# lis-epfl/apg_trajectory_tracking

Hardware: AMD Instinct MI355X
Metric: env-steps/sec (fwd+bwd through dynamics), quad horizon=10 batch=65536 (higher is better)
Workload: dtype f32; 1 GPU; quadrotor concurrent rollout fwd+bwd (dynamics + quad_mpc_loss + adjoint), BASELINE configs[1]; batch_per_gpu=65536, global_batch=65536, horizon=10, layout=packed, buffer_sets=20, input_bytes_all_sets=587202560, grad_state0=False, loss_mode=deferred, launch=hip-graph replays of the K steps, <= 1000 steps per graph, replays=3, parallelism=batch-sharded x1, no data-path collective

## Files before the change

apg_trajectory_tracking_amd/csrc/mlp_concurrent.hip:

```cpp
#include "mlp_concurrent_fwd.h"

namespace apg {
namespace {
template <bool ROWS>
__global__ __launch_bounds__(kThreads) void mlp_concurrent_bwd_tm_kernel(WgArgs A) {
  extern __shared__ __attribute__((aligned(16))) float lds_f[];
  char *lds = reinterpret_cast<char *>(lds_f);
  const int lane = threadIdx.x & 63, hi = lane >> 5, row = lane & 31;
  const int wave = __builtin_amdgcn_readfirstlane(threadIdx.x >> 6);
  const int b0 = blockIdx.x * kTrajPerBlock;
  const int b = b0 + wave * 32 + row;
  const int B = A.B;
  const bool live = b < B;
  const unsigned pN = (unsigned)B * 4u;
  const Planes Pact(A.acts, kActPlanes, pN), Pdz(A.d_zout, kNA, pN);
  const unsigned vb = live ? (unsigned)b * 4u : kDead;
  const unsigned vr = live ? vb + (hi ? 4u * pN : 0u) : kDead;
  const unsigned wcol = (unsigned)(b0 + wave * 32) * 4u;
  const unsigned vt = (unsigned)row * pN + (unsigned)hi * 16u;
  const int nw = B - (b0 + wave * 32);
  float *part = A.part + (size_t)blockIdx.x * kSlotsTm * 1024;
  char *lane_blk = lds + lane * 4;
  TmMeta &meta = *reinterpret_cast<TmMeta *>(lds + tMeta);
  bool bad = false;
// ... 210 lines not shown
      if (hi == 0)
        __builtin_nontemporal_store(
            bad ? __builtin_nanf("") : __builtin_amdgcn_ldexpf(sb, e_ - kPreD),
            bias_part + bias_id * 64 + 32 * mb + row);
      split16(v, 0, ad[mb]);
    }
  };
  auto layer64 = [&](f32x16 (&dl)[2], f32x16 (&nx)[2], int e_, int tab, int x_plane,
                     int region, int bias_id, int next_plane, int phase) {
    Op16 x[4];
    const int ex = scaled_split64(dl, x);
    Op16 ad[2][2];
    transposed_operands(x, ex, e_, bias_id, ad);
#pragma unroll
    for (int nb = 0; nb < 2; ++nb) {
      float xv[16];
      tx.get(xv);
      tx.load(Pact, vt, (unsigned)(nb == 0 ? x_plane + 32 : next_plane) * pN + wcol);
      Op16 bx[2];
      split16(xv, -kPreX, bx);
#pragma unroll
      for (int mb = 0; mb < 2; ++mb) {
        f32x16 acc;
#pragma unroll
        for (int i = 0; i < 16; ++i) acc[i] = 0.f;
#pragma unroll
        for (int kk = 0; kk < 2; ++kk) acc = mma3(ad[mb][kk], bx[kk], acc);
        add_block(lane_blk + region + (2 * nb + mb) * 4096, acc);
      }
      if (nb == 0) load_hv(x_plane);
    }
    zero(nx);
    dense64T_16(nx, x, L16, 0, tab);
#pragma unroll
    for (int rb = 0; rb < 2; ++rb)
#pragma unroll
      for (int i = 0; i < 16; ++i)
        nx[rb][i] = __builtin_amdgcn_ldexpf(nx[rb][i], ex) * (1.f - hv[rb][i] * hv[rb][i]);
    post(nx, phase + 1);
  };
  const int e3 = wg_exp(meta.dmax[1], bad);
  layer64(d, e, e3, w3, pH2, tRB, 1, pH1, 1);
  __syncthreads();
  flush_region(lds, tRB, 4 * 1024, part + sFc3 * 1024, e3, true, bad);
  zero_region(lds, tF1a, tRA - tF1a);
  const int e2 = wg_exp(meta.dmax[2], bad);
  layer64(e, d, e2, w2, pH1, tRA, 2, pX1, 2);
  __syncthreads();
  flush_region(lds, tRA, 4 * 1024, part + sFc2 * 1024, e2, false, bad);

  const int e1 = wg_exp(meta.dmax[3], bad);
  const int es = e1 + ns, ec = e1 + nc;
  {
    Op16 x1s[4];
    const int ex1 = scaled_split64(d, x1s);
    Op16 ad[2][2];
    transposed_operands(x1s, ex1, e1, 3, ad);
    Op16 bfeat[2], binr[3][2];
    if (ROWS) {
      const int bw = b0 + wave * 32 + row;
      const long long r_ = A.index[bw < B ? bw : B - 1];
      const unsigned rf = row_offset(r_, A.n_rows, A.ld_feat);
      const unsigned ri = row_offset(r_, A.n_rows, A.ld_in_ref);
      const auto sf = __builtin_amdgcn_make_buffer_rsrc(const_cast<float *>(A.r_feat), 0,
                                                        (int)A.bytes_feat, 0x00020000);
      const auto si = __builtin_amdgcn_make_buffer_rsrc(const_cast<float *>(A.r_in_ref), 0,
                                                        (int)A.bytes_in_ref, 0x00020000);
      float v[16];
      const auto rows_block = [&](__amdgpu_buffer_rsrc_t rs, unsigned rbase, int col, bool on) {
#pragma unroll
        for (int g = 0; g < 4; ++g)
#pragma unroll
          for (int c = 0; c < 4; ++c) {
            const unsigned a0 = (unsigned)__builtin_amdgcn_readlane((int)rbase, c + 8 * g),
                           a1 = (unsigned)__builtin_amdgcn_readlane((int)rbase, c + 8 * g + 4);
            const unsigned a = hi ? a1 : a0;
            const unsigned off = on && a != kDead ? a + 4u * (unsigned)col : kDead;
            v[4 * g + c] = __builtin_bit_cast(
                float, __builtin_amdgcn_raw_buffer_load_b32(rs, (int)off, 0, APG_PLANES_LD_AUX));
          }
      };
      rows_block(sf, rf, row, row < kNF);
#pragma unroll
      for (int i = 0; i < 16; ++i) v[i] = row == kNF ? 1.f : v[i];
      split16(v, ff - kPreX, bfeat);
#pragma unroll
      for (int jb = 0; jb < 3; ++jb) {
        rows_block(si, ri, 32 * jb + row, 32 * jb + row < kH * kRD);
        split16(v, fi - kPreXc, binr[jb]);
      }
    } else {
      TBlock tf;
      tf.load(Pact, row < kNF ? vt : kDead, (unsigned)pFeat * pN + wcol);
      float v[16];
      tf.get(v);
#pragma unroll
      for (int i = 0; i < 16; ++i) v[i] = row == kNF ? 1.f : v[i];
      split16(v, ff - kPreX, bfeat);
#pragma unroll
      for (int jb = 0; jb < 3; ++jb) {
        tf.load(Pact, 32 * jb + row < kH * kRD ? vt : kDead,
                (unsigned)(pInr + 32 * jb) * pN + wcol);
        tf.get(v);
        split16(v, fi - kPreXc, binr[jb]);
      }
    }
// ... 382 lines not shown
```

apg_trajectory_tracking_amd/csrc/mlp_rollout.hip:

```cpp
#include "mlp_common.h"
#include "quad_flight.h"

namespace apg {
namespace {
template <bool XMAX, bool LEGACY = false>
__global__ __launch_bounds__(kThreads) void mlp_rollout_fwd_kernel(FwdArgs A) {
  extern __shared__ __attribute__((aligned(16))) float lds[];
  fill_lds(lds, A.tables, kCfLds);
  const LdsView16 L16(lds, threadIdx.x & 63);
  const int lane = threadIdx.x & 63, hi = lane >> 5;
  const LdsView L(lds, lane);
  const int wave = __builtin_amdgcn_readfirstlane(threadIdx.x >> 6);
  const int b = (blockIdx.x * (kThreads / 64) + wave) * 32 + (lane & 31);
  const int B = A.B;
  const bool live = b < B;
  const bool st_lo = live && hi == 0;
  const unsigned pitchB = (unsigned)B * 4u, pitchN = pitchB * kH;
  const QuadConst c = A.c;
  const Planes Ps0(A.state0, 12, pitchB), Pin(A.in_ref, 2 * kH * kRD, pitchB);
  const Planes Pst(A.states, kH * 12, pitchB), Pac(A.actions, kH * 4, pitchB);
  const Planes Pfe(A.feat, kNF, pitchN), Px1(A.x1, kN1, pitchN);
  const Planes Ph(A.h, 3 * kW, pitchN), Pmk(A.mask, 5, pitchN);
  const unsigned vb = live ? (unsigned)b * 4u : kDead;
  const unsigned vb_lo = st_lo ? vb : kDead;

  float s[12];
#pragma unroll
  for (int i = 0; i < 12; ++i) s[i] = Ps0.ld(vb, i * pitchB);
  const unsigned vwin = live ? vb + (hi ? 4u * pitchB : 0u) : kDead;
  float w[kH][5];
#pragma unroll
  for (int r = 0; r < kH; ++r)
#pragma unroll
    for (int j = 0; j < 5; ++j) w[r][j] = Pin.ld(vwin, (r * kRD + j) * pitchB);
  float wmax_raw = 0.f;
  if (XMAX) {
#pragma unroll
    for (int r = 0; r < kH; ++r)
#pragma unroll
      for (int j = 0; j < 5; ++j) wmax_raw = fmaxf(wmax_raw, fabsf(w[r][j]));
  }

#pragma unroll 1
  for (int k = 0; k < kH; ++k) {
    const unsigned pB = opaque(pitchB), pN = opaque(pitchN);
    const unsigned col = (unsigned)b * 4u + (unsigned)k * pitchB;
    const unsigned vn = live ? col : kDead;
    const unsigned vn_lo = st_lo ? col : kDead;
    const unsigned vr = live ? col + (hi ? 4u * pitchN : 0u) : kDead;
    const unsigned vc = live ? col + (hi ? 32u * pitchN : 0u) : kDead;
    const unsigned vm = live ? col + (hi ? pitchN : 0u) : kDead;
    const Trig t = make_trig(&s[3]);
    float feat[kNF];
    quad_features(s, t, feat);
#pragma unroll
    for (int j = 0; j < kNF; ++j) Pfe.st(vn_lo, j * pN, feat[j]);
    float xm_c = 0.f;
    if (XMAX) {
      float xm_f = 0.f;
#pragma unroll
      for (int j = 0; j < kNF; ++j) xm_f = fmaxf(xm_f, fabsf(feat[j]));
      const float xm_i = wmax_raw + (hi ? 0.f : fmaxf(fmaxf(fabsf(s[0]), fabsf(s[1])), fabsf(s[2])));
      const float rf = wave_fmax(xm_f), ri = wave_fmax(xm_i);
      if (lane == 0) {
        float *q = A.xmax + ((size_t)(blockIdx.x * (kThreads / 64) + wave) * kH + k) * 4;
        q[1] = rf, q[2] = ri;
      }
    }

    f32x16 u[2], a[2];
    init_bias(u, L, hTbs);
    {
      float v[8];
#pragma unroll
      for (int j = 0; j < 8; ++j)
        v[j] = hi ? (8 + j < kNF ? feat[8 + j < kNF ? 8 + j : 0] : 0.f) : feat[j];
      const Op16 x = split8(v);
      u[0] = mma3(L16.A(hA, nS + 0), x, u[0]);
      u[1] = mma3(L16.A(hA, nS + 1), x, u[1]);
    }
    float sub[3] = {hi ? 0.f : s[0], hi ? 0.f : s[1], hi ? 0.f : s[2]};
    if (LEGACY) {
#pragma unroll
      for (int r = 0; r < kH; ++r)
#pragma unroll
        for (int j = 0; j < 3; ++j) w[r][j] -= sub[j];
      sub[0] = sub[1] = sub[2] = 0.f;
    }
    init_bias(a, L, hTb1);
    unsigned mbits[3] = {0u, 0u, 0u};
#pragma unroll
    for (int pp = 0; pp < kNP / 2; ++pp) {
      float rv[24];
      unsigned ws[4][5];
#pragma unroll
      for (int r = 0; r < 4; ++r)
#pragma unroll
        for (int j = 0; j < 5; ++j) {
          const float xv = j < 3 ? w[2 * pp + r][j] - sub[j] : w[2 * pp + r][j];
          const _Float16 vh = (_Float16)xv, vl = (_Float16)(xv - (float)vh);
          const h16x2 pr = {vh, vl};
          ws[r][j] = __builtin_bit_cast(unsigned, pr);
        }
#pragma unroll
// ... 224 lines not shown
    for (int sft = 32; sft >= 1; sft >>= 1) sum = fmaxf(sum, __shfl_xor(sum, sft, 64));
    if ((t & 63) == 0) wmax[t >> 6] = sum;
    __syncthreads();
    if (t < 2) {
      const float m = t ? fmaxf(fmaxf(wmax[1], wmax[2]), wmax[3]) : wmax[0];
      A.dst[kCfLds + kArTabFloats + t] =
          m > 0.f && m < 3.0e38f ? (float)__builtin_amdgcn_frexp_expf(m) : 0.f;
    }
    return;
  }
  if ((int)blockIdx.x < fwd_blocks) {
    pack_cfwd(A, blockIdx.x * blockDim.x + threadIdx.x, fwd_blocks * blockDim.x);
    return;
  }
  const int tid = (blockIdx.x - fwd_blocks) * blockDim.x + threadIdx.x;
  const int T = (gridDim.x - 1 - fwd_blocks) * blockDim.x;
  float *dstf = A.dst + kCfLds;
  unsigned *dst = reinterpret_cast<unsigned *>(dstf);
  for (int idx = tid; idx < aBlocks * 64 * 4; idx += T) {
    const int q = idx & 3, l = (idx >> 2) & 63, n = idx >> 8;
    const float w0 = car_weight(A.pol, n, l & 31, 2 * q, l >> 5);
    const float w1 = car_weight(A.pol, n, l & 31, 2 * q + 1, l >> 5);
    unsigned h, lo;
    split_pair(w0, w1, h, lo);
    dst[(gA + n * kBlock16) / 4 + l * 4 + q] = h;
    dst[(gA + n * kBlock16 + 1024) / 4 + l * 4 + q] = lo;
  }
  const ApgMlpPolicy &p = A.pol;
  for (int idx = tid; idx < 256; idx += T) {
    const int hi = idx & 1, i = (idx >> 1) & 15, rb = (idx >> 5) & 1, j = idx >> 6;
    dstf[gTo + idx] = p.w_out[j * kW + rb * 32 + rrow(i) + 4 * hi];
  }
  for (int idx = tid; idx < kNC * 3; idx += T) {
    const int ch = idx / 3, q = idx % 3;
    dstf[gAq + idx] = p.conv_w[ch * 27 + q * 3] + p.conv_w[ch * 27 + q * 3 + 1] +
                      p.conv_w[ch * 27 + q * 3 + 2];
  }
}

struct ArTmArgs {
  const float *state0, *states, *actions, *ref, *in_ref;
  const float *feat, *x1, *h;
  const unsigned *mask;
  float *loss_partials;
  float *part;
  float *grad_state0;
  const float *tables;
  const float *xmax;
  QuadConst c;
  ApgQuadLossWeights w;
  int B, ref_cols, vel_col;
};

__device__ __forceinline__ void ar_sink(const f32x16 &acc) {
  float s_ = 0.f;
#pragma unroll
  for (int i = 0; i < 16; ++i) s_ += acc[i];
  asm volatile("" ::"v"(s_));
}
__device__ __forceinline__ void ar_barrier() {
  if (APG_AR_KNOCKOUT & 16) return;
  __syncthreads();
}

struct ArMeta {
  unsigned dmax[5][8];
};
static_assert(rMeta + (int)sizeof(ArMeta) <= kLdsAll, "LDS map");

__global__ __launch_bounds__(kThreads) void mlp_rollout_bwd_tm_kernel(ArTmArgs A) {
  extern __shared__ __attribute__((aligned(16))) float lds_f[];
  char *lds = reinterpret_cast<char *>(lds_f);
  const int lane = threadIdx.x & 63, hi = lane >> 5, row = lane & 31;
  const int wave = __builtin_amdgcn_readfirstlane(threadIdx.x >> 6);
  const int b0 = blockIdx.x * kTrajPerBlock;
  const int b = b0 + wave * 32 + row;
  const int B = A.B;
  const bool live = b < B, st_lo = live && hi == 0;
  const unsigned pitchB = (unsigned)B * 4u, pitchN = pitchB * kH;
  const QuadConst c = A.c;
  const Planes Ps0(A.state0, 12, pitchB), Pst(A.states, kH * 12, pitchB);
  const Planes Pac(A.actions, kH * 4, pitchB), Prf(A.ref, kH * A.ref_cols, pitchB);
  const Planes Pin(A.in_ref, 2 * kH * kRD, pitchB);
  const Planes Pfe(A.feat, kNF, pitchN), Px1(A.x1, kN1, pitchN), Ph(A.h, 3 * kW, pitchN);
  const Planes Pmk(A.mask, 5, pitchN);
  const unsigned vb = live ? (unsigned)b * 4u : kDead;
  const unsigned wcolB = (unsigned)(b0 + wave * 32) * 4u;
  const unsigned vtN = (unsigned)row * pitchN + (unsigned)hi * 16u;
  const unsigned vtB = (unsigned)row * pitchB + (unsigned)hi * 16u;
  const __amdgpu_buffer_rsrc_t part = __builtin_amdgcn_make_buffer_rsrc(
      A.part + (size_t)blockIdx.x * kSlotsTm * 1024, 0, kSlotsTm * 4096, 0x00020000);
  char *lane_blk = lds + lane * 4;
  ArMeta &meta = *reinterpret_cast<ArMeta *>(lds + rMeta);
  const int ns = (int)A.tables[kArTabFloats];
  bool bad = false;

  zero_region(lds, rX, rMeta - rX);
  {
    const u32x4 z = {0u, 0u, 0u, 0u};
#pragma unroll
    for (int m = 0; m < kSlotsTm * 256; m += kThreads)
      __builtin_amdgcn_raw_buffer_store_b128(z, part, (int)(threadIdx.x * 16u), m * 16, 0);
  }
  fill_lds_issue(lds_f, A.tables, kArTabFloats);
  asm volatile("s_waitcnt vmcnt(0)" ::: "memory");
  __syncthreads();
  const LdsView16 L16(lds, lane);
  const LdsView L(lds_f, lane);
  float lam[12];
#pragma unroll
  for (int i = 0; i < 12; ++i) lam[i] = 0.f;
  float loss = 0.f;
  int rg = rX, ro = rY;
  int e5 = 0, ecv = 0;
  TBlock tx, tx2;
  const auto post = [&](const f32x16 (&v)[2], int phase) {
    unsigned am = 0u;
#pragma unroll
    for (int rb = 0; rb < 2; ++rb)
#pragma unroll
      for (int i = 0; i < 16; ++i) am = umax_abs(am, v[rb][i]);
    am = wave_umax(am);
    if (lane == 0) meta.dmax[phase][wave] = am;
  };
  const unsigned bias_soff = (unsigned)(uBias + (wave >> 2)) * 4096u + (unsigned)(wave & 3) * 1024u;
  const auto flush_tail = [&]() {
    flush_add<4 * 1024>(lds, rg, part, (sFc1 + 10) * 4096, e5, bad);
    flush_add<1024>(lds, rConv, part, uConv * 4096, ecv, bad, kFixConv);
  };

#pragma unroll 1
  for (int k = kH - 1; k >= 0; --k) {
    const unsigned pB = (APG_AR_KNOCKOUT & 64) ? 256u : opaque(pitchB), pN = opaque(pitchN);
    const unsigned col = (unsigned)b * 4u + (unsigned)k * pitchB;
    const unsigned vn = live ? ((APG_AR_KNOCKOUT & 64) ? (unsigned)lane * 4u : col) : kDead;
    const unsigned wcolN = wcolB + (unsigned)k * pB;
    u32x4 ident[2];
    {
      int lane_o = lane;
      asm volatile("" : "+v"(lane_o));
      ident_operands(lane_o, ident);
    }
    float dz[4];
    unsigned m0 = 0u;
    f32x16 d[2], e[2];
    float x3[2][16];
    {
      float sn[12], sc[12], a[4], rp[3], rv[3];
#pragma unroll
      for (int i = 0; i < 12; ++i) {
        sn[i] = Pst.ld(vb, (k * 12 + i) * pB);
        sc[i] = k > 0 ? Pst.ld(vb, ((k - 1) * 12 + i) * pB) : Ps0.ld(vb, i * pB);
      }
#pragma unroll
      for (int j = 0; j < 4; ++j) a[j] = Pac.ld(vb, (k * 4 + j) * pB);
#pragma unroll
      for (int i = 0; i < 3; ++i) {
        rp[i] = Prf.ld(vb, (k * A.ref_cols + i) * pB);
        rv[i] = Prf.ld(vb, (k * A.ref_cols + A.vel_col + i) * pB);
      }
      tx.load(Ph, vtN, (unsigned)(2 * kW) * pN + wcolN);
      tx2.load(Ph, vtN, (unsigned)(2 * kW + 32) * pN + wcolN);
      __builtin_amdgcn_sched_barrier(0);
      float lp = 0.f, lv = 0.f, lw = 0.f, lr = 0.f;
#pragma unroll
      for (int i = 0; i < 3; ++i) {
        const float dp = sn[i] - rp[i], dv = sn[6 + i] - rv[i], wn = sn[9 + i];
        lp += dp * dp, lv += dv * dv, lw += wn * wn;
        lam[i] += 2.f * A.w.pos * dp;
        lam[6 + i] += 2.f * A.w.vel * dv;
        lam[9 + i] += 2.f * A.w.av * wn;
      }
      const float da0 = a[0] - 0.5f;
      float ga[4];
      ga[0] = 2.f * A.w.thrust * da0;
#pragma unroll
      for (int j = 1; j < 4; ++j) {
        const float dd = a[j] - 0.5f;
        lr += dd * dd;
        ga[j] = 2.f * A.w.rates * dd;
      }
      loss += A.w.pos * lp + A.w.vel * lv + A.w.av * lw + A.w.rates * lr +
              A.w.thrust * da0 * da0;
      const Trig t = make_trig(&sc[3]);
      quad_step_adjoint(lam, ga, a[0], &sc[9], c, t);
#pragma unroll
      for (int j = 0; j < 4; ++j) {
        dz[j] = ga[j] * a[j] * (1.f - a[j]);
        m0 = umax_abs(m0, dz[j]);
      }
    }
    tx.get(x3[0]);
    tx2.get(x3[1]);
    tx.load(Ph, vtN, (unsigned)kW * pN + wcolN);
#pragma unroll
    for (int rb = 0; rb < 2; ++rb) {
      Op16 bx[2];
      split16(x3[rb], -kPreX, bx);
      const f32x16 hf = to_feature_major(bx, ident);
#pragma unroll
      for (int i = 0; i < 16; ++i) {
        float v = 0.f;
#pragma unroll
        for (int j = 0; j < 4; ++j)
          v = fmaf(L.T(gTo + ((j * 2 + rb) * 16 + i) * 2), dz[j], v);
        const float h3 = __builtin_amdgcn_ldexpf(hf[i], -kPreX);
        d[rb][i] = v * (1.f - h3 * h3);
      }
    }
    m0 = wave_umax(m0);
    if (lane == 0) meta.dmax[0][wave] = m0;
    post(d, 1);
    unsigned mc = 0u, mf = 0x3f800000u , mi = 0u;
    {
      const unsigned *q = reinterpret_cast<const unsigned *>(A.xmax) +
                          ((size_t)blockIdx.x * (kThreads / 64) * kH + k) * 4;
#pragma unroll
      for (int w8 = 0; w8 < kThreads / 64; ++w8) {
        mc = q[w8 * kH * 4] > mc ? q[w8 * kH * 4] : mc;
        mf = q[w8 * kH * 4 + 1] > mf ? q[w8 * kH * 4 + 1] : mf;
        mi = q[w8 * kH * 4 + 2] > mi ? q[w8 * kH * 4 + 2] : mi;
      }
    }
    const int fc = bits_exp(mc, bad, true), ff = bits_exp(mf, bad, true),
              fi = bits_exp(mi, bad, true);
    ar_barrier();
    flush_tail();
    { const int r_ = rg; rg = ro, ro = r_; }

    const int e0 = wg_exp(meta.dmax[0], bad), e3 = wg_exp(meta.dmax[1], bad);
    {
      float v8[8];
#pragma unroll
      for (int j = 0; j < 8; ++j)
        v8[j] = (hi == 0 && j < 4) ? __builtin_amdgcn_ldexpf(dz[j < 4 ? j : 0], kPreD - e0) : 0.f;
      const Op16 x0 = split8(v8);
      u32x4 idz;
#pragma unroll
      for (int q = 0; q < 4; ++q)
        idz[q] = (8 * hi + 2 * q == row ? 0x3c00u : 0u) |
                 (8 * hi + 2 * q + 1 == row ? 0x3c000000u : 0u);
      f32x16 tzv;
#pragma unroll
      for (int i = 0; i < 16; ++i) tzv[i] = 0.f;
      tzv = mfma16(x0.l, idz, tzv);
      tzv = mfma16(x0.h, idz, tzv);
      float tz[16], sb = 0.f;
#pragma unroll
      for (int i = 0; i < 16; ++i) {
        tz[i] = tzv[i];
        sb += tz[i];
      }
      sb += other_half(sb);
      if (hi == 0 && row < 4)
        gadd(part, (unsigned)row * 4u, bias_soff,
             bad ? __builtin_nanf("") : __builtin_amdgcn_ldexpf(sb, e0 - kPreD));
      Op16 az[2];
      split16(tz, 0, az);
#pragma unroll
      for (int nb = 0; nb < 2; ++nb) {
        Op16 bx[2];
        split16(x3[nb], -kPreX, bx);
        f32x16 acc;
#pragma unroll
        for (int i = 0; i < 16; ++i) acc[i] = 0.f;
#pragma unroll
        for (int kk = 0; kk < 2; ++kk) acc = mma3(az[kk], bx[kk], acc);
        if (hi == 0) {
#pragma unroll
          for (int i = 0; i < 4; ++i) lds_add(lds + rHead + (i * 64 + 32 * nb + row) * 4, acc[i]);
        }
      }
    }
    const auto transposed_operands = [&](const Op16 (&x)[4], int ex, int e_, int bias_id,
                                         Op16 (&ad)[2][2]) {
      int E[16];
      texp(ex, hi, E);
#pragma unroll
      for (int mb = 0; mb < 2; ++mb) {
        const Op16 pr[2] = {x[2 * mb], x[2 * mb + 1]};
// ... 3 lines not shown
        for (int i = 0; i < 16; ++i) {
          v[i] = __builtin_amdgcn_ldexpf(tz[i], E[i] - e_ + kPreD);
          sb += v[i];
        }
        sb += other_half(sb);
        if (bias_id >= 0 && hi == 0)
          gadd(part, (unsigned)(bias_id * 64 + 32 * mb + row) * 4u, bias_soff,
               bad ? __builtin_nanf("") : __builtin_amdgcn_ldexpf(sb, e_ - kPreD));
        split16(v, 0, ad[mb]);
      }
    };
    const auto layer64 = [&](f32x16 (&dl)[2], f32x16 (&nx)[2], int e_, int tab, const Planes &X,
                             int x_plane, const Planes &Xn, int next_plane, int bias_id,
                             int phase, char *rb) {
      Op16 x[4];
      const int ex = scaled_split64(dl, x);
      Op16 ad[2][2];
      transposed_operands(x, ex, e_, bias_id, ad);
#pragma unroll
      for (int nb = 0; nb < 2; ++nb) {
        float xv[16];
        tx.get(xv);
        if (nb == 0) tx.load(X, vtN, (unsigned)(x_plane + 32) * pN + wcolN);
        else tx.load(Xn, vtN, (unsigned)next_plane * pN + wcolN);
        Op16 bx[2];
        split16(xv, -kPreX, bx);
#pragma unroll
        for (int mb = 0; mb < 2; ++mb) {
          if (APG_AR_KNOCKOUT & 2) break;
          f32x16 acc;
#pragma unroll
          for (int i = 0; i < 16; ++i) acc[i] = 0.f;
#pragma unroll
          for (int kk = 0; kk < 2; ++kk) acc = mma3(ad[mb][kk], bx[kk], acc);
          if (APG_AR_KNOCKOUT & 4) ar_sink(acc); else
          add_block(rb + (2 * nb + mb) * 4096, acc);
        }
#pragma unroll
        for (int i = 0; i < 16; ++i) nx[nb][i] = 0.f;
#pragma unroll
        for (int kb = 0; kb < 4; ++kb) nx[nb] = mma3(L16.A(gA, tab + 4 * nb + kb), x[kb], nx[nb]);
        const f32x16 hf = to_feature_major(bx, ident);
#pragma unroll
        for (int i = 0; i < 16; ++i) {
          const float hx = __builtin_amdgcn_ldexpf(hf[i], -kPreX);
          nx[nb][i] = __builtin_amdgcn_ldexpf(nx[nb][i], ex) * (1.f - hx * hx);
        }
        __builtin_amdgcn_sched_barrier(0);
      }
      post(nx, phase + 1);
    };
    layer64(d, e, e3, a3, Ph, kW, Ph, 0, 1, 1, lane_blk + rg);
    ar_barrier();
    if (threadIdx.x < 4 * 64) {
      const int idx = threadIdx.x;
      int *p = reinterpret_cast<int *>(lds + rHead) + idx;
      const int q = *p;
      *p = 0;
      gadd(part, (unsigned)((idx >> 6) * 64 + (idx & 31)) * 4u,
           (sOut + 2 * ((idx >> 5) & 1)) * 4096,
           bad ? __builtin_nanf("") : __builtin_amdgcn_ldexpf((float)q, e0 - kFix));
    }
    flush_add<4 * 1024>(lds, rg, part, sFc3 * 4096, e3, bad);
    { const int r_ = rg; rg = ro, ro = r_; }

    const int e2 = wg_exp(meta.dmax[2], bad);
    layer64(e, d, e2, a2, Ph, 0, Px1, 0, 2, 2, lane_blk + rg);
    ar_barrier();
    flush_add<4 * 1024>(lds, rg, part, sFc2 * 4096, e2, bad);
    { const int r_ = rg; rg = ro, ro = r_; }

    const int e1 = wg_exp(meta.dmax[3], bad);
    const int es = e1 + ns;
    Op16 x1s[4];
    const int ex1 = scaled_split64(d, x1s);
    Op16 ad[2][2];
    transposed_operands(x1s, ex1, e1, 3, ad);
    const auto fc1_blocks = [&](const Op16 (&bx)[2], char *blk) {
#pragma unroll
      for (int mb = 0; mb < 2; ++mb) {
        if (APG_AR_KNOCKOUT & 2) break;
        f32x16 acc;
#pragma unroll
        for (int i = 0; i < 16; ++i) acc[i] = 0.f;
#pragma unroll
        for (int kk = 0; kk < 2; ++kk) acc = mma3(ad[mb][kk], bx[kk], acc);
        if (APG_AR_KNOCKOUT & 4) ar_sink(acc); else
        add_block(blk + mb * 4096, acc);
      }
    };
    Op16 bfeat[2];
    {
      {
        TBlock tf;
        tf.load(Pfe, row < kNF ? vtN : kDead, wcolN);
        float v[16];
        get_clamped(tf, v, ff);
#pragma unroll
        for (int i = 0; i < 16; ++i) v[i] = row == kNF ? 1.f : v[i];
        split16(v, ff - kPreX, bfeat);
      }
#pragma unroll
      for (int nb = 0; nb < 2; ++nb) {
        float xv[16];
        tx.get(xv);
        tx.load(Px1, vtN, (unsigned)(32 * (nb + 1)) * pN + wcolN);
        Op16 bx[2];
        split16(xv, -kPreX, bx);
        fc1_blocks(bx, lane_blk + rg + 2 * nb * 4096);
#pragma unroll
        for (int i = 0; i < 16; ++i) e[nb][i] = 0.f;
#pragma unroll
        for (int kb = 0; kb < 4; ++kb) e[nb] = mma3(L16.A(gA, a1s + 4 * nb + kb), x1s[kb], e[nb]);
        const f32x16 hf = to_feature_major(bx, ident);
#pragma unroll
        for (int i = 0; i < 16; ++i) {
          const float hx = __builtin_amdgcn_ldexpf(hf[i], -kPreX);
          e[nb][i] = __builtin_amdgcn_ldexpf(e[nb][i], ex1) * (1.f - hx * hx);
        }
        __builtin_amdgcn_sched_barrier(0);
      }
    }
    __builtin_amdgcn_sched_barrier(0);
    {
      float sc[12];
#pragma unroll
      for (int i = 0; i < 12; ++i)
        sc[i] = k > 0 ? Pst.ld(vb, ((k - 1) * 12 + i) * pB) : Ps0.ld(vb, i * pB);
      f32x16 f;
#pragma unroll
      for (int i = 0; i < 16; ++i) f[i] = 0.f;
      Op16 xs[4];
      const int exs = scaled_split64(e, xs);
      {
        Op16 as[2][2];
        transposed_operands(xs, exs, es, -1, as);
#pragma unroll
        for (int nb = 0; nb < 2; ++nb) {
          f32x16 acc;
#pragma unroll
          for (int i = 0; i < 16; ++i) acc[i] = 0.f;
#pragma unroll
          for (int kk = 0; kk < 2; ++kk) acc = mma3(as[nb][kk], bfeat[kk], acc);
          if (row < 16) {
            char *q = lds + rg + 4 * 4096 + nb * 2048 + (hi * 16 + row) * 4;
#pragma unroll
            for (int i = 0; i < 16; ++i) lds_add2(q + i * 128, q + 4096 + i * 128, acc[i], kFix);
          }
        }
      }
#pragma unroll
      for (int kb = 0; kb < 4; ++kb) f = mma3(L16.A(gA, aS + kb), xs[kb], f);
      const Trig t = make_trig(&sc[3]);
      float dfeat[kNF], gs[12];
#pragma unroll
      for (int i = 0; i < 8; ++i) {
        const float own = __builtin_amdgcn_ldexpf(f[i], exs), oth = other_half(own);
        dfeat[rrow(i)] = hi ? oth : own;
        if (rrow(i) + 4 < kNF) dfeat[rrow(i) + 4 < kNF ? rrow(i) + 4 : 0] = hi ? own : oth;
      }
      quad_features_adjoint(sc, t, dfeat, gs);
#pragma unroll
      for (int i = 0; i < 12; ++i) lam[i] += gs[i];
    }
    __builtin_amdgcn_sched_barrier(0);
    {
      unsigned mw[5];
#pragma unroll
      for (int eb = 0; eb < 5; ++eb) mw[eb] = Pmk.ldu(vn, eb * pN);
      float dpos[3] = {0.f, 0.f, 0.f};
      unsigned cm = 0u;
#pragma unroll 1
      for (int eb = 0; eb < 5; ++eb) {
        const char *tb = L16.b0 + gA + (a1c + 4 * eb) * kBlock16;
        f32x16 y;
#pragma unroll
        for (int i = 0; i < 16; ++i) y[i] = 0.f;
#pragma unroll
        for (int kb = 0; kb < 4; ++kb) {
          Op16 w;
          w.h = *reinterpret_cast<const u32x4 *>(tb + kb * kBlock16);
          w.l = *reinterpret_cast<const u32x4 *>(tb + kb * kBlock16 + 1024);
          y = mma3(w, x1s[kb], y);
        }
        const unsigned mwe = eb == 0 ? mw[0] : eb == 1 ? mw[1] : eb == 2 ? mw[2]
                             : eb == 3 ? mw[3] : mw[4];
        const unsigned mws = hi ? mwe >> 4 : mwe;
#pragma unroll
        for (int g = 0; g < 4; ++g) {
          float sg = 0.f;
#pragma unroll
          for (int ii = 0; ii < 4; ++ii) {
            const int i = 4 * g + ii;
            const float yv = ((mws >> rrow(i)) & 1u) ? __builtin_amdgcn_ldexpf(y[i], ex1) : 0.f;
            cm = umax_abs(cm, yv);
            sg += yv;
          }
#pragma unroll
          for (int q = 0; q < 3; ++q)
            dpos[q] = fmaf(lds_f[L.o_0 + gAq + (eb * 4 + g) * 3 + q], sg, dpos[q]);
        }
      }
#pragma unroll
      for (int q = 0; q < 3; ++q) lam[q] -= dpos[q] + other_half(dpos[q]);
      cm = wave_umax(cm);
      if (lane == 0) meta.dmax[4][wave] = cm;
    }
    ar_barrier();
    flush_add<4 * 1024>(lds, rg, part, sFc1 * 4096, e1, bad);
#pragma unroll
    for (int nb = 0; nb < 2; ++nb) {
      const int r_ = threadIdx.x, at = (r_ >> 5) * 64 + 32 * ((r_ >> 4) & 1) + (r_ & 15);
      int *q = reinterpret_cast<int *>(lds + rg + 4 * 4096) + nb * 512 + r_;
      const double v = (double)q[0] + (double)q[1024] * (1.0 / (double)(1 << kFix));
      q[0] = 0, q[1024] = 0;
      gadd(part, (unsigned)at * 4u, (sSin + nb) * 4096,
           bad ? __builtin_nanf("") : __builtin_amdgcn_ldexpf((float)v, es + ff - kFix));
    }
    { const int r_ = rg; rg = ro, ro = r_; }

    const int ec = wg_exp(meta.dmax[4], bad);
    Op16 binr[3][2];
    {
      const Planes Pp = k > 0 ? Pst : Ps0;
      const unsigned pbase = k > 0 ? (unsigned)((k - 1) * 12) * pB : 0u;
#pragma unroll
      for (int jb = 0; jb < 3; ++jb) {
        const int j = 32 * jb + row;
        TBlock tf, tp;
        tf.load(Pin, j < kH * kRD ? vtB : kDead, (unsigned)(k * kRD + 32 * jb) * pB + wcolB);
        tp.load(Pp, (j < kH * kRD && j % kRD < 3) ? (unsigned)(j % kRD) * pitchB + (unsigned)hi * 16u
                                                 : kDead, pbase + wcolB);
        float v[16], pv[16];
        tf.get(v);
        tp.get(pv);
        const float lim = __builtin_amdgcn_ldexpf(1.f, fi);
#pragma unroll
        for (int i = 0; i < 16; ++i)
          v[i] = __builtin_amdgcn_fmed3f(v[i] - pv[i], -lim, lim);
        split16(v, fi - kPreXc, binr[jb]);
      }
    }
#pragma unroll 1
    for (int eb = 0; eb < 5; ++eb) {
      if (eb == 3) {
        ar_barrier();
        flush_add<6 * 1024>(lds, rg, part, (sFc1 + 4) * 4096, e1 + fc, bad);
        const int r_ = rg; rg = ro, ro = r_;
      }
      float xv[16];
      get_clamped(tx, xv, fc);
      if (eb < 4) tx.load(Px1, vtN, (unsigned)(kW + 32 * (eb + 1)) * pN + wcolN);
      int row_e = row, hi_e = hi;
      asm volatile("" : "+v"(row_e), "+v"(hi_e));
      {
        Op16 bx[2];
        split16(xv, fc - kPreX, bx);
        fc1_blocks(bx, lane_blk + rg + 2 * (eb < 3 ? eb : eb - 3) * 4096);
      }
      __builtin_amdgcn_sched_barrier(0);
      const char *tb = L16.b0 + gA + (a1c + 4 * eb) * kBlock16;
      f32x16 tt;
#pragma unroll
      for (int i = 0; i < 16; ++i) tt[i] = 0.f;
#pragma unroll
      for (int kb = 0; kb < 4; ++kb) {
        Op16 w;
        w.h = *reinterpret_cast<const u32x4 *>(tb + kb * kBlock16);
        w.l = *reinterpret_cast<const u32x4 *>(tb + kb * kBlock16 + 1024);
        tt = mma3(x1s[kb], w, tt);
      }
      int E1[16];
      texp(ex1, hi, E1);
      float v[16], sum = 0.f;
#pragma unroll
      for (int i = 0; i < 16; ++i) {
        v[i] = xv[i] > 0.f ? __builtin_amdgcn_ldexpf(tt[i], E1[i] - ec) : 0.f;
        sum += v[i];
      }
      char *cblk = lds + rConv + ((4 * (eb >> 1)) * 64 + 32 * (eb & 1)) * 4;
      sum += other_half(sum);
      sum += __builtin_bit_cast(float, __builtin_amdgcn_update_dpp(
          0, __builtin_bit_cast(int, sum), 0x111 , 0xf, 0xf, true)) *
             ((row_e & 7) >= 1 ? 1.f : 0.f);
      sum += __builtin_bit_cast(float, __builtin_amdgcn_update_dpp(
          0, __builtin_bit_cast(int, sum), 0x112 , 0xf, 0xf, true)) *
             ((row_e & 7) >= 2 ? 1.f : 0.f);
      sum += __builtin_bit_cast(float, __builtin_amdgcn_update_dpp(
          0, __builtin_bit_cast(int, sum), 0x114 , 0xf, 0xf, true)) *
             ((row_e & 7) >= 4 ? 1.f : 0.f);
      if (hi_e == 0 && (row_e & 7) == 7)
        gadd(part, (unsigned)(32 + 4 * eb + (row_e >> 3)) * 4u, bias_soff,
             bad ? __builtin_nanf("") : __builtin_amdgcn_ldexpf(sum, ec));
      Op16 ac[2];
      split16(v, -kPreDc, ac);
#pragma unroll
      for (int jb = 0; jb < 3; ++jb) {
        if (APG_AR_KNOCKOUT & 8) break;
        f32x16 acc;
#pragma unroll
        for (int i = 0; i < 16; ++i) acc[i] = 0.f;
#pragma unroll
        for (int kk = 0; kk < 2; ++kk) acc = mma3(ac[kk], binr[jb][kk], acc);
#pragma unroll
        for (int cc = 0; cc < 4; ++cc) {
          const int q = 32 * jb + row_e - kRD * (cc + 4 * hi_e);
          if (q >= 0 && q < 27) {
#pragma unroll
            for (int g = 0; g < 4; ++g) lds_add(cblk + (g * 64 + q) * 4, acc[4 * g + cc]);
          }
        }
      }
    }
    e5 = e1 + fc, ecv = ec + fi;
  }
  ar_barrier();
  flush_tail();
  if (st_lo && A.grad_state0)
#pragma unroll
    for (int i = 0; i < 12; ++i) A.grad_state0[(size_t)i * B + b] = lam[i];
  write_wave_partial(A.loss_partials, st_lo ? loss : 0.f);
}

}
}

using namespace apg;

extern "C" {

int apg_quad_mlp_workspace_floats(void) {
  return (kCfLds > kCbLds ? kCfLds : kCbLds) + kLearntFloats;
}

int apg_quad_mlp_loss_partials_count(int B) {
  return B <= 0 ? 0 : ((B + kTrajPerBlock - 1) / kTrajPerBlock) * (kThreads / kWave);
}

static int mlp_rollout_fwd(const float *state0, const float *in_ref, float dt,
                           const ApgQuadParams *params, const ApgMlpPolicy *policy, int B, int H,
                           float *states, float *actions, float *feat, float *x1, float *h,
                           unsigned *relu_mask, float *workspace, apg_stream_t stream,
                           bool legacy_inplace_ref);

int apg_quad_mlp_rollout_fwd(const float *state0, const float *in_ref, float dt,
                             const ApgQuadParams *params,
                             const ApgMlpPolicy *policy, int B, int H,
                             float *states, float *actions, float *feat,
                             float *x1, float *h, unsigned *relu_mask,
                             float *workspace, apg_stream_t stream) {
  return mlp_rollout_fwd(state0, in_ref, dt, params, policy, B, H, states, actions, feat, x1, h,
                         relu_mask, workspace, stream, false);
}

int apg_quad_mlp_rollout_fwd_inplace_ref(const float *state0, const float *in_ref, float dt,
                                         const ApgQuadParams *params,
                                         const ApgMlpPolicy *policy, int B, int H,
                                         float *states, float *actions, float *feat,
                                         float *x1, float *h, unsigned *relu_mask,
                                         float *workspace, apg_stream_t stream) {
  return mlp_rollout_fwd(state0, in_ref, dt, params, policy, B, H, states, actions, feat, x1, h,
                         relu_mask, workspace, stream, true);
}

static int mlp_rollout_fwd(const float *state0, const float *in_ref, float dt,
                           const ApgQuadParams *params, const ApgMlpPolicy *policy, int B, int H,
                           float *states, float *actions, float *feat, float *x1, float *h,
                           unsigned *relu_mask, float *workspace, apg_stream_t stream,
                           bool legacy_inplace_ref) {
  if (int e = check_mlp(params, policy, B, H)) return e;
// ... 186 lines not shown
```

apg_trajectory_tracking_amd/csrc/policy_tm.h:

```cpp
#pragma once
#include "policy_mfma16.h"

namespace apg {

constexpr int kTmThreads = 512;

__device__ __forceinline__ float wave_fmax(float v) {
#pragma unroll
  for (int s = 32; s >= 1; s >>= 1) v = fmaxf(v, __shfl_xor(v, s, 64));
  return v;
}

constexpr int kFix = 22, kFixConv = 19;
constexpr int kPreD = 11, kPreX = kFix - kPreD, kPreDc = 10, kPreXc = kFixConv - kPreDc;
constexpr unsigned kInfBits = 0x7f800000u;
__device__ __forceinline__ unsigned umax_abs(unsigned m, float v) {
  const unsigned b = __builtin_bit_cast(unsigned, v) & 0x7fffffffu;
  return b > m ? b : m;
}
__device__ __forceinline__ unsigned wave_umax(unsigned v) {
#pragma unroll
  for (int s = 32; s >= 1; s >>= 1) {
    const unsigned o = (unsigned)__shfl_xor((int)v, s, 64);
    v = o > v ? o : v;
  }
  return (unsigned)__builtin_amdgcn_readfirstlane((int)v);
}
__device__ __forceinline__ int bits_exp(unsigned a, bool &bad, bool nonneg_floor) {
  if (a >= kInfBits) {
    bad = true;
    return 0;
  }
  const int e = a ? __builtin_amdgcn_frexp_expf(__builtin_bit_cast(float, a)) : 0;
  return nonneg_floor && e < 0 ? 0 : e;
}

typedef float f32x4_ __attribute__((ext_vector_type(4)));
typedef int i32x4_ __attribute__((ext_vector_type(4)));

#if !defined(APG_EXPERIMENT_BUILD) && defined(APG_AR_KNOCKOUT)
#error "experiment macro in a product build (variants: tools/build_policy_variant.sh)"
#endif
#ifndef APG_AR_KNOCKOUT
#define APG_AR_KNOCKOUT 0
#endif

struct TBlock {
  u32x4 q[4];
  __device__ __forceinline__ void load(const Planes &X, unsigned voff, unsigned soff) {
    if (APG_AR_KNOCKOUT & 32) {
      voff = (threadIdx.x & 31u) * 64u + ((threadIdx.x & 32u) ? 16u : 0u);
      soff = 0u;
    }
    if (APG_AR_KNOCKOUT & 128) {
      voff = voff == kDead ? kDead : (threadIdx.x & 63u) * 16u;
#pragma unroll
      for (int g = 0; g < 4; ++g)
        q[g] = __builtin_amdgcn_raw_buffer_load_b128(X.rsrc, (int)voff, (int)(soff + 1024 * g),
                                                     APG_PLANES_LD_AUX);
      return;
    }
#pragma unroll
    for (int g = 0; g < 4; ++g)
      q[g] = __builtin_amdgcn_raw_buffer_load_b128(X.rsrc, (int)voff, (int)(soff + 32 * g),
                                                   APG_PLANES_LD_AUX);
  }
  __device__ __forceinline__ void get(float (&v)[16]) const {
#pragma unroll
    for (int g = 0; g < 4; ++g) {
      const f32x4_ f = __builtin_bit_cast(f32x4_, q[g]);
#pragma unroll
      for (int c = 0; c < 4; ++c) v[4 * g + c] = f[c];
    }
  }
};

__device__ __forceinline__ void split16(const float (&v)[16], int e, Op16 (&o)[2]) {
#pragma unroll
  for (int kk = 0; kk < 2; ++kk) {
    float w8[8];
#pragma unroll
    for (int j = 0; j < 8; ++j) w8[j] = __builtin_amdgcn_ldexpf(v[8 * kk + j], -e);
    o[kk] = split8(w8);
  }
}

#if !defined(APG_EXPERIMENT_BUILD) && (defined(APG_TM_KNOCKOUT) || defined(APG_TM_PLAIN_PARTIALS))
#error "experiment macro in a product build (variants: tools/build_policy_variant.sh)"
#endif
#ifndef APG_TM_KNOCKOUT
#define APG_TM_KNOCKOUT 0
#endif
__device__ __forceinline__ void lds_add(char *p, float v, int fix = kFix) {
  if (APG_TM_KNOCKOUT & 1) {
    __hip_atomic_fetch_add(reinterpret_cast<float *>(p), v, __ATOMIC_RELAXED,
                           __HIP_MEMORY_SCOPE_WORKGROUP);
    return;
  }
  (void)fix;
  const int q = (int)__builtin_rintf(v);
  __hip_atomic_fetch_add(reinterpret_cast<int *>(p), q, __ATOMIC_RELAXED,
                         __HIP_MEMORY_SCOPE_WORKGROUP);
}

__device__ __forceinline__ void lds_add2(char *hi, char *lo, float v, int fix = kFixConv) {
  const float s_ = v, qh = __builtin_rintf(s_);
  __hip_atomic_fetch_add(reinterpret_cast<int *>(hi), (int)qh, __ATOMIC_RELAXED,
                         __HIP_MEMORY_SCOPE_WORKGROUP);
  __hip_atomic_fetch_add(reinterpret_cast<int *>(lo),
                         (int)__builtin_rintf(__builtin_amdgcn_ldexpf(s_ - qh, fix)),
                         __ATOMIC_RELAXED, __HIP_MEMORY_SCOPE_WORKGROUP);
}

__device__ __forceinline__ void add_block(char *blk_lane, const f32x16 &acc) {
#pragma unroll
  for (int i = 0; i < 16; ++i) lds_add(blk_lane + i * 256, acc[i]);
}

__device__ __forceinline__ void flush_region(char *lds, int off, int floats, float *dst, int e,
                                             bool rezero, bool bad, int fix = kFix) {
  const i32x4_ z = {0, 0, 0, 0};
  for (int idx = threadIdx.x; idx < floats / 4; idx += kTmThreads) {
    i32x4_ *p = reinterpret_cast<i32x4_ *>(lds + off) + idx;
    const i32x4_ q = *p;
    f32x4_ v;
#pragma unroll
    for (int c = 0; c < 4; ++c)
      v[c] = bad ? __builtin_nanf("") : __builtin_amdgcn_ldexpf((float)q[c], e - fix);
#ifdef APG_TM_PLAIN_PARTIALS
    reinterpret_cast<f32x4_ *>(dst)[idx] = v;
#else
    __builtin_nontemporal_store(v, reinterpret_cast<f32x4_ *>(dst) + idx);
#endif
    if (rezero) *p = z;
  }
}

__device__ __forceinline__ void zero_region(char *lds, int off, int bytes) {
  const f32x4_ z = {0.f, 0.f, 0.f, 0.f};
  for (int idx = threadIdx.x; idx < bytes / 16; idx += kTmThreads)
    reinterpret_cast<f32x4_ *>(lds + off)[idx] = z;
}

__device__ __forceinline__ int wg_exp(const unsigned (&slots)[8], bool &bad) {
  unsigned a = slots[0];
#pragma unroll
  for (int w = 1; w < 8; ++w) a = slots[w] > a ? slots[w] : a;
  return bits_exp(a, bad, false);
}

__device__ __forceinline__ void get_clamped(const TBlock &t, float (&v)[16], int f) {
  t.get(v);
  const float lim = __builtin_amdgcn_ldexpf(1.f, f);
#pragma unroll
  for (int i = 0; i < 16; ++i) v[i] = __builtin_amdgcn_fmed3f(v[i], -lim, lim);
}

__device__ __forceinline__ void texp(int ex, int hi, int (&E)[16]) {
  const _Float16 hx = (_Float16)(float)ex;
  u32x4 a = {0u, 0u, 0u, 0u}, o = {0u, 0u, 0u, 0u};
  a[0] = hi ? 0u : (unsigned)__builtin_bit_cast(unsigned short, hx);
  o[0] = hi ? 0u : 0x3c00u;
  f32x16 z;
#pragma unroll
  for (int i = 0; i < 16; ++i) z[i] = 0.f;
  z = mfma16(a, o, z);
#pragma unroll
  for (int i = 0; i < 16; ++i) E[i] = (int)z[i];
}

__device__ __forceinline__ void gadd(__amdgpu_buffer_rsrc_t r, unsigned voff, unsigned soff,
                                     float v) {
  if (APG_AR_KNOCKOUT & 1) return;
  __builtin_amdgcn_raw_ptr_buffer_atomic_fadd_f32(v, r, (int)voff, (int)soff, 0);
}
// ... 41 lines not shown
```

Baseline: 76.20 billion env-steps/s.

## Cut register pressure in rollout backward by rematerializing per-step values inside loop

Moves lane, wave, address, and LDS-view values into the time-step loop so they are recomputed each iteration instead of held live across it. Kernel-argument constants (quad constants, loss weights, plane pointers) are now read on demand from the kernarg segment. Optimization barriers and sched_barriers pin live ranges. wave_umax is rewritten to use DPP row ops plus a readlane instead of xor shuffles. The aim is to avoid VGPR spills and shorten reductions, at the cost of extra recomputation and more fragile, compiler-dependent scheduling.

```diff
diff --git a/apg_trajectory_tracking_amd/csrc/mlp_concurrent.hip b/apg_trajectory_tracking_amd/csrc/mlp_concurrent.hip
--- a/apg_trajectory_tracking_amd/csrc/mlp_concurrent.hip
+++ b/apg_trajectory_tracking_amd/csrc/mlp_concurrent.hip
@@ -286,6 +286,12 @@
   const int e1 = wg_exp(meta.dmax[3], bad);
   const int es = e1 + ns, ec = e1 + nc;
   {
+    int tid_o = threadIdx.x;
+    asm volatile("" : "+v"(tid_o));
+    const int lane = tid_o & 63, hi = lane >> 5, row = lane & 31;
+    const unsigned vt = (unsigned)row * pN + (unsigned)hi * 16u;
+    char *lane_blk = lds + lane * 4;
+    const LdsView16 L16(lds, lane);
     Op16 x1s[4];
     const int ex1 = scaled_split64(d, x1s);
     Op16 ad[2][2];
diff --git a/apg_trajectory_tracking_amd/csrc/mlp_rollout.hip b/apg_trajectory_tracking_amd/csrc/mlp_rollout.hip
--- a/apg_trajectory_tracking_amd/csrc/mlp_rollout.hip
+++ b/apg_trajectory_tracking_amd/csrc/mlp_rollout.hip
@@ -47,9 +47,9 @@
     const unsigned col = (unsigned)b * 4u + (unsigned)k * pitchB;
     const unsigned vn = live ? col : kDead;
     const unsigned vn_lo = st_lo ? col : kDead;
-    const unsigned vr = live ? col + (hi ? 4u * pitchN : 0u) : kDead;
-    const unsigned vc = live ? col + (hi ? 32u * pitchN : 0u) : kDead;
-    const unsigned vm = live ? col + (hi ? pitchN : 0u) : kDead;
+    const unsigned vr = live ? col + (hi ? 4u * pN : 0u) : kDead;
+    const unsigned vc = live ? col + (hi ? 32u * pN : 0u) : kDead;
+    const unsigned vm = live ? col + (hi ? pN : 0u) : kDead;
     const Trig t = make_trig(&s[3]);
     float feat[kNF];
     quad_features(s, t, feat);
@@ -380,6 +380,20 @@
   int B, ref_cols, vel_col;
 };
 
+typedef const __attribute__((address_space(4))) char *KArgPtr;
+template <class T>
+__device__ __forceinline__ T karg(KArgPtr p, size_t off) {
+  return *reinterpret_cast<const __attribute__((address_space(4))) T *>(p + off);
+}
+template <class S>
+__device__ __forceinline__ S karg_floats(KArgPtr p, size_t off) {
+  static_assert(sizeof(S) % 4 == 0, "a struct of floats");
+  struct F { float f[sizeof(S) / 4]; } f;
+#pragma unroll
+  for (size_t i = 0; i < sizeof(S) / 4; ++i) f.f[i] = karg<float>(p, off + 4 * i);
+  return __builtin_bit_cast(S, f);
+}
+
 __device__ __forceinline__ void ar_sink(const f32x16 &acc) {
   float s_ = 0.f;
 #pragma unroll
@@ -389,6 +403,11 @@
 __device__ __forceinline__ void ar_barrier() {
   if (APG_AR_KNOCKOUT & 16) return;
   __syncthreads();
+}
+
+__device__ __forceinline__ void pin12(float (&lam)[12]) {
+#pragma unroll
+  for (int i = 0; i < 12; ++i) asm volatile("" : "+v"(lam[i]));
 }
 
 struct ArMeta {
@@ -399,27 +418,16 @@
 __global__ __launch_bounds__(kThreads) void mlp_rollout_bwd_tm_kernel(ArTmArgs A) {
   extern __shared__ __attribute__((aligned(16))) float lds_f[];
   char *lds = reinterpret_cast<char *>(lds_f);
-  const int lane = threadIdx.x & 63, hi = lane >> 5, row = lane & 31;
-  const int wave = __builtin_amdgcn_readfirstlane(threadIdx.x >> 6);
+  const int wave0 = __builtin_amdgcn_readfirstlane(threadIdx.x >> 6);
   const int b0 = blockIdx.x * kTrajPerBlock;
-  const int b = b0 + wave * 32 + row;
   const int B = A.B;
-  const bool live = b < B, st_lo = live && hi == 0;
   const unsigned pitchB = (unsigned)B * 4u, pitchN = pitchB * kH;
-  const QuadConst c = A.c;
+  const KArgPtr ka0 = (KArgPtr)__builtin_amdgcn_kernarg_segment_ptr();
   const Planes Ps0(A.state0, 12, pitchB), Pst(A.states, kH * 12, pitchB);
   const Planes Pac(A.actions, kH * 4, pitchB), Prf(A.ref, kH * A.ref_cols, pitchB);
-  const Planes Pin(A.in_ref, 2 * kH * kRD, pitchB);
-  const Planes Pfe(A.feat, kNF, pitchN), Px1(A.x1, kN1, pitchN), Ph(A.h, 3 * kW, pitchN);
-  const Planes Pmk(A.mask, 5, pitchN);
-  const unsigned vb = live ? (unsigned)b * 4u : kDead;
-  const unsigned wcolB = (unsigned)(b0 + wave * 32) * 4u;
-  const unsigned vtN = (unsigned)row * pitchN + (unsigned)hi * 16u;
-  const unsigned vtB = (unsigned)row * pitchB + (unsigned)hi * 16u;
+  const Planes Px1(A.x1, kN1, pitchN), Ph(A.h, 3 * kW, pitchN);
   const __amdgpu_buffer_rsrc_t part = __builtin_amdgcn_make_buffer_rsrc(
       A.part + (size_t)blockIdx.x * kSlotsTm * 1024, 0, kSlotsTm * 4096, 0x00020000);
-  char *lane_blk = lds + lane * 4;
-  ArMeta &meta = *reinterpret_cast<ArMeta *>(lds + rMeta);
   const int ns = (int)A.tables[kArTabFloats];
   bool bad = false;
 
@@ -433,8 +441,6 @@
   fill_lds_issue(lds_f, A.tables, kArTabFloats);
   asm volatile("s_waitcnt vmcnt(0)" ::: "memory");
   __syncthreads();
-  const LdsView16 L16(lds, lane);
-  const LdsView L(lds_f, lane);
   float lam[12];
 #pragma unroll
   for (int i = 0; i < 12; ++i) lam[i] = 0.f;
@@ -442,23 +448,42 @@
   int rg = rX, ro = rY;
   int e5 = 0, ecv = 0;
   TBlock tx, tx2;
-  const auto post = [&](const f32x16 (&v)[2], int phase) {
-    unsigned am = 0u;
-#pragma unroll
-    for (int rb = 0; rb < 2; ++rb)
-#pragma unroll
-      for (int i = 0; i < 16; ++i) am = umax_abs(am, v[rb][i]);
-    am = wave_umax(am);
-    if (lane == 0) meta.dmax[phase][wave] = am;
-  };
-  const unsigned bias_soff = (unsigned)(uBias + (wave >> 2)) * 4096u + (unsigned)(wave & 3) * 1024u;
-  const auto flush_tail = [&]() {
+  const auto flush_tail = [&](char *lds) {
     flush_add<4 * 1024>(lds, rg, part, (sFc1 + 10) * 4096, e5, bad);
     flush_add<1024>(lds, rConv, part, uConv * 4096, ecv, bad, kFixConv);
   };
 
 #pragma unroll 1
   for (int k = kH - 1; k >= 0; --k) {
+    const int wave = (int)opaque((unsigned)wave0);
+    KArgPtr ka = ka0;
+    asm volatile("" : "+s"(ka));
+    char *const lds_all = lds;
+    char *const lds = lds_all + opaque(0u);
+    float *const lds_f = reinterpret_cast<float *>(lds);
+    ArMeta &meta = *reinterpret_cast<ArMeta *>(lds + rMeta);
+    const unsigned wcolB = (unsigned)(b0 + wave * 32) * 4u;
+    const unsigned bias_soff = (unsigned)(uBias + (wave >> 2)) * 4096u + (unsigned)(wave & 3) * 1024u;
+    int tid_o = threadIdx.x;
+    asm volatile("" : "+v"(tid_o));
+    const int lane = tid_o & 63, hi = lane >> 5, row = lane & 31;
+    const int b = b0 + wave * 32 + row;
+    const bool live = b < B;
+    const unsigned vb = live ? (unsigned)b * 4u : kDead;
+    const unsigned vtN = (unsigned)row * pitchN + (unsigned)hi * 16u;
+    const unsigned vtB = (unsigned)row * pitchB + (unsigned)hi * 16u;
+    char *lane_blk = lds + lane * 4;
+    const LdsView16 L16(lds, lane);
+    const LdsView L(lds_f, lane);
+    const auto post = [&](const f32x16 (&v)[2], int phase) {
+      unsigned am = 0u;
+#pragma unroll
+      for (int rb = 0; rb < 2; ++rb)
+#pragma unroll
+        for (int i = 0; i < 16; ++i) am = umax_abs(am, v[rb][i]);
+      am = wave_umax(am);
+      if (lane == 0) meta.dmax[phase][wave] = am;
+    };
     const unsigned pB = (APG_AR_KNOCKOUT & 64) ? 256u : opaque(pitchB), pN = opaque(pitchN);
     const unsigned col = (unsigned)b * 4u + (unsigned)k * pitchB;
     const unsigned vn = live ? ((APG_AR_KNOCKOUT & 64) ? (unsigned)lane * 4u : col) : kDead;
@@ -475,6 +500,8 @@
     float x3[2][16];
     {
       float sn[12], sc[12], a[4], rp[3], rv[3];
+      const QuadConst c = karg_floats<QuadConst>(ka, offsetof(ArTmArgs, c));
+      const ApgQuadLossWeights w = karg_floats<ApgQuadLossWeights>(ka, offsetof(ArTmArgs, w));
 #pragma unroll
       for (int i = 0; i < 12; ++i) {
         sn[i] = Pst.ld(vb, (k * 12 + i) * pB);
@@ -495,29 +522,32 @@
       for (int i = 0; i < 3; ++i) {
         const float dp = sn[i] - rp[i], dv = sn[6 + i] - rv[i], wn = sn[9 + i];
         lp += dp * dp, lv += dv * dv, lw += wn * wn;
-        lam[i] += 2.f * A.w.pos * dp;
-        lam[6 + i] += 2.f * A.w.vel * dv;
-        lam[9 + i] += 2.f * A.w.av * wn;
+        lam[i] += 2.f * w.pos * dp;
+        lam[6 + i] += 2.f * w.vel * dv;
+        lam[9 + i] += 2.f * w.av * wn;
       }
       const float da0 = a[0] - 0.5f;
       float ga[4];
-      ga[0] = 2.f * A.w.thrust * da0;
+      ga[0] = 2.f * w.thrust * da0;
 #pragma unroll
       for (int j = 1; j < 4; ++j) {
         const float dd = a[j] - 0.5f;
         lr += dd * dd;
-        ga[j] = 2.f * A.w.rates * dd;
-      }
-      loss += A.w.pos * lp + A.w.vel * lv + A.w.av * lw + A.w.rates * lr +
-              A.w.thrust * da0 * da0;
+        ga[j] = 2.f * w.rates * dd;
+      }
+      loss += w.pos * lp + w.vel * lv + w.av * lw + w.rates * lr +
+              w.thrust * da0 * da0;
+      asm volatile("" : "+v"(loss));
       const Trig t = make_trig(&sc[3]);
       quad_step_adjoint(lam, ga, a[0], &sc[9], c, t);
+      pin12(lam);
 #pragma unroll
       for (int j = 0; j < 4; ++j) {
         dz[j] = ga[j] * a[j] * (1.f - a[j]);
         m0 = umax_abs(m0, dz[j]);
       }
     }
+    __builtin_amdgcn_sched_barrier(0);
     tx.get(x3[0]);
     tx2.get(x3[1]);
     tx.load(Ph, vtN, (unsigned)kW * pN + wcolN);
@@ -533,7 +563,10 @@
         for (int j = 0; j < 4; ++j)
           v = fmaf(L.T(gTo + ((j * 2 + rb) * 16 + i) * 2), dz[j], v);
         const float h3 = __builtin_amdgcn_ldexpf(hf[i], -kPreX);
-        d[rb][i] = v * (1.f - h3 * h3);
+        float dv = v * (1.f - h3 * h3);
+        asm volatile("" : "+v"(dv));
+        d[rb][i] = dv;
+        if ((i & 3) == 3) __builtin_amdgcn_sched_barrier(0);
       }
     }
     m0 = wave_umax(m0);
@@ -541,7 +574,8 @@
     post(d, 1);
     unsigned mc = 0u, mf = 0x3f800000u , mi = 0u;
     {
-      const unsigned *q = reinterpret_cast<const unsigned *>(A.xmax) +
+      const unsigned *q = reinterpret_cast<const unsigned *>(
+                              karg<const float *>(ka, offsetof(ArTmArgs, xmax))) +
                           ((size_t)blockIdx.x * (kThreads / 64) * kH + k) * 4;
 #pragma unroll
       for (int w8 = 0; w8 < kThreads / 64; ++w8) {
@@ -553,7 +587,7 @@
     const int fc = bits_exp(mc, bad, true), ff = bits_exp(mf, bad, true),
               fi = bits_exp(mi, bad, true);
     ar_barrier();
-    flush_tail();
+    flush_tail(lds);
     { const int r_ = rg; rg = ro, ro = r_; }
 
     const int e0 = wg_exp(meta.dmax[0], bad), e3 = wg_exp(meta.dmax[1], bad);
@@ -663,8 +697,8 @@
     };
     layer64(d, e, e3, a3, Ph, kW, Ph, 0, 1, 1, lane_blk + rg);
     ar_barrier();
-    if (threadIdx.x < 4 * 64) {
-      const int idx = threadIdx.x;
+    if (wave < 4) {
+      const int idx = tid_o;
       int *p = reinterpret_cast<int *>(lds + rHead) + idx;
       const int q = *p;
       *p = 0;
@@ -703,6 +737,7 @@
     Op16 bfeat[2];
     {
       {
+        const Planes Pfe(karg<const float *>(ka, offsetof(ArTmArgs, feat)), kNF, pitchN);
         TBlock tf;
         tf.load(Pfe, row < kNF ? vtN : kDead, wcolN);
         float v[16];
@@ -773,9 +808,11 @@
       quad_features_adjoint(sc, t, dfeat, gs);
 #pragma unroll
       for (int i = 0; i < 12; ++i) lam[i] += gs[i];
+      pin12(lam);
     }
     __builtin_amdgcn_sched_barrier(0);
     {
+      const Planes Pmk(karg<const unsigned *>(ka, offsetof(ArTmArgs, mask)), 5, pitchN);
       unsigned mw[5];
 #pragma unroll
       for (int eb = 0; eb < 5; ++eb) mw[eb] = Pmk.ldu(vn, eb * pN);
@@ -833,6 +870,7 @@
     const int ec = wg_exp(meta.dmax[4], bad);
     Op16 binr[3][2];
     {
+      const Planes Pin(karg<const float *>(ka, offsetof(ArTmArgs, in_ref)), 2 * kH * kRD, pitchB);
       const Planes Pp = k > 0 ? Pst : Ps0;
       const unsigned pbase = k > 0 ? (unsigned)((k - 1) * 12) * pB : 0u;
 #pragma unroll
@@ -926,7 +964,9 @@
     e5 = e1 + fc, ecv = ec + fi;
   }
   ar_barrier();
-  flush_tail();
+  flush_tail(lds);
+  const int lane = threadIdx.x & 63, b = b0 + wave0 * 32 + (lane & 31);
+  const bool st_lo = b < B && lane < 32;
   if (st_lo && A.grad_state0)
 #pragma unroll
     for (int i = 0; i < 12; ++i) A.grad_state0[(size_t)i * B + b] = lam[i];
diff --git a/apg_trajectory_tracking_amd/csrc/policy_tm.h b/apg_trajectory_tracking_amd/csrc/policy_tm.h
--- a/apg_trajectory_tracking_amd/csrc/policy_tm.h
+++ b/apg_trajectory_tracking_amd/csrc/policy_tm.h
@@ -18,13 +18,19 @@
   const unsigned b = __builtin_bit_cast(unsigned, v) & 0x7fffffffu;
   return b > m ? b : m;
 }
+template <int kCtrl, int kRows>
+__device__ __forceinline__ unsigned umax_dpp(unsigned v) {
+  const unsigned o = (unsigned)__builtin_amdgcn_update_dpp((int)v, (int)v, kCtrl, kRows, 0xf, false);
+  return o > v ? o : v;
+}
 __device__ __forceinline__ unsigned wave_umax(unsigned v) {
-#pragma unroll
-  for (int s = 32; s >= 1; s >>= 1) {
-    const unsigned o = (unsigned)__shfl_xor((int)v, s, 64);
-    v = o > v ? o : v;
-  }
-  return (unsigned)__builtin_amdgcn_readfirstlane((int)v);
+  v = umax_dpp<0xb1, 0xf>(v);
+  v = umax_dpp<0x4e, 0xf>(v);
+  v = umax_dpp<0x141, 0xf>(v);
+  v = umax_dpp<0x140, 0xf>(v);
+  v = umax_dpp<0x142, 0xa>(v);
+  v = umax_dpp<0x143, 0xc>(v);
+  return (unsigned)__builtin_amdgcn_readlane((int)v, 63);
 }
 __device__ __forceinline__ int bits_exp(unsigned a, bool &bad, bool nonneg_floor) {
   if (a >= kInfBits) {
@@ -120,7 +126,9 @@
 __device__ __forceinline__ void flush_region(char *lds, int off, int floats, float *dst, int e,
                                              bool rezero, bool bad, int fix = kFix) {
   const i32x4_ z = {0, 0, 0, 0};
-  for (int idx = threadIdx.x; idx < floats / 4; idx += kTmThreads) {
+  int t0 = threadIdx.x;
+  asm volatile("" : "+v"(t0));
+  for (int idx = t0; idx < floats / 4; idx += kTmThreads) {
     i32x4_ *p = reinterpret_cast<i32x4_ *>(lds + off) + idx;
     const i32x4_ q = *p;
     f32x4_ v;
```

Result: no change. 75.92 billion env-steps/s (-0.4%).
